# CVMI-Lab/DODA

Hardware: AMD Instinct MI355X
Metric: active-voxels/sec fwd+bwd SparseConv U-Net, ScanNet 2cm (higher is better)
Workload: dtype bf16; 1 GPU; cfgs/scannet SparseConv U-Net training step (voxel pooling + fwd + CE + bwd + SGD), 2 cm voxels, 4 scenes/GPU x ~150000 active voxels, random-init weights; global_batch=4, voxels_per_gpu=601279, points_per_gpu=781042, parallelism=dp1, n_classes=20, grad_sync=deferred multi-layer wgrad + bucketed all-reduce, collectives=none (single process), prefetch_gate=off, grad_exchange=no process group

## Files before the change

doda_amd/csrc/spconv_wdma.hip:

```cpp
#include "tilebook.hpp"
#include "spconv_common.hpp"
#include "wgrad_common.hpp"
#include <stdlib.h>
#include <type_traits>
#include <string.h>

namespace {

constexpr int WD_WAVES = 16;
constexpr int WD_ROWS_BYTES = (TB_UMAX + 1) * 32;
constexpr int WD_LIDX_BYTES = TB_LIDX_BYTES;
constexpr int WD_DY_BYTES = TB_T * 32;
constexpr int WD_UNITS_BYTES = 2 * TB_K * 256 * 4;
constexpr int WD_BUF_BYTES = (WD_ROWS_BYTES + WD_LIDX_BYTES + WD_DY_BYTES) > WD_UNITS_BYTES ? (WD_ROWS_BYTES + WD_LIDX_BYTES + WD_DY_BYTES)
                                                                                           : WD_UNITS_BYTES;
static_assert(WD_LIDX_BYTES % 1024 == 0, "whole DMA pieces");
constexpr int WD_UNITS = 2 * TB_K;
constexpr int WD_MAX_UNITS = (WD_UNITS + WD_WAVES - 1) / WD_WAVES;
constexpr int WD_MAX_JOBS = 16;
static_assert(WD_BUF_BYTES % 16 == 0 && 2 * WD_BUF_BYTES + 64 <= 160 * 1024, "two tile buffers per CU");
static_assert(WD_UNITS * 256 * 4 <= WD_BUF_BYTES, "the final exchange re-uses ONE tile buffer (the other may be a DMA target)");

struct WdJob { const void *x, *dy; float *part; unsigned x_stride, dy_stride; int first_rank, pad; };
struct WdJobs { int n; WdJob j[WD_MAX_JOBS]; };

__device__ __forceinline__ u32x4 wd_rsrc(const void *p, unsigned bytes) {
    const unsigned long long a = (unsigned long long)p;
    u32x4 r;
    r[0] = (unsigned)a;
    r[1] = (unsigned)(a >> 32) & 0xffffu;
    r[2] = bytes;
    r[3] = 0x00020000u;
    return r;
}
__device__ __forceinline__ void wd_dma16(unsigned lds_base, unsigned voff, const u32x4 &rs) {
    unsigned keep;
    asm volatile("s_mov_b32 %0, m0\n\t"
                 "s_mov_b32 m0, %1\n\t"
                 "s_nop 0\n\t"
                 "buffer_load_dwordx4 %2, %3, 0 offen lds\n\t"
                 "s_mov_b32 m0, %0"
                 : "=&s"(keep) : "s"(lds_base), "v"(voff), "s"(rs) : "memory");
}
__device__ __forceinline__ void wd_aload128(u32x4 &dst, unsigned voff, const u32x4 &rs) {
    asm volatile("buffer_load_dwordx4 %0, %1, %2, 0 offen" : "=v"(dst) : "v"(voff), "s"(rs) : "memory");
}
template <int TAG = 0>
__device__ __forceinline__ s16x4 wd_tr_b64(unsigned addr) {
    s16x4 v;
    asm volatile("ds_read_b64_tr_b16 %0, %1 ; %2" : "=v"(v) : "v"(addr), "n"(TAG) : "memory");
    return v;
}
__global__ __launch_bounds__(1024) void wgrad_dma16(const WdJobs jobs, const int32_t *__restrict__ tbl,
                                                    int ld, int n, const TileBookView tb) {
    __shared__ __attribute__((aligned(16))) unsigned char smem[2 * WD_BUF_BYTES];
    const int tid = threadIdx.x, wid = __builtin_amdgcn_readfirstlane(tid >> 6);
    const int lane = tid & 63, i = lane & 15, g = lane >> 4;
    const u32x4 rs_ul = wd_rsrc(tb.ulist, (unsigned)tb.nt * (unsigned)TB_UMAX * 4u);
    const u32x4 rs_li = wd_rsrc(tb.lidx, (unsigned)tb.nt * (unsigned)TB_LIDX_BYTES);

    const int G = gridDim.x, nt = tb.nt;
    const int rank = (int)(blockIdx.x & 7) * (G >> 3) + (int)(blockIdx.x >> 3);
    const long long N = (long long)jobs.n * nt;
    const int start = (int)((long long)rank * N / G), n_items = (int)((long long)(rank + 1) * N / G) - start;
    if (n_items == 0) return;

    if (tid < 4) reinterpret_cast<u32x4 *>(smem + (tid >> 1) * WD_BUF_BYTES)[tid & 1] = (u32x4){0u, 0u, 0u, 0u};

    const unsigned smem_base = (unsigned)(uintptr_t)smem;
    const unsigned src_half = (unsigned)(lane & 1) * 16u;
    const int w8 = wid & 7, kb = (wid >> 3) * 2;
    struct Where { int job; unsigned tile; bool ok; };
    auto where = [&](int item) {
        Where q;
        q.ok = item < n_items;
        const int gid = start + (q.ok ? item : 0);
        q.job = gid / nt;
        q.tile = (unsigned)(gid - q.job * nt);
        return q;
    };
    auto issue_list = [&](const Where &q, u32x2 &rid) {
        asm volatile("buffer_load_dwordx2 %0, %1, %2, 0 offen" : "=v"(rid)
                     : "v"(q.ok ? q.tile * (unsigned)(TB_UMAX * 4) + (unsigned)((w8 * 32 + (lane >> 1)) * 4 + kb) * 4u : OOB), "s"(rs_ul)
                     : "memory");
    };
    auto issue_rows = [&](const Where &q, int item, int k, const u32x2 &rid) {
        const unsigned buf = smem_base + (unsigned)(item & 1) * (unsigned)WD_BUF_BYTES;
        const unsigned xs = jobs.j[q.job].x_stride;
        const u32x4 rs_x = wd_rsrc(jobs.j[q.job].x, (unsigned)n * xs - (xs - 32u));
        if (!q.ok || __builtin_amdgcn_readfirstlane((int)rid[k]) < 0) return;
        wd_dma16(buf + 32u + (unsigned)(((kb + k) * 8 + w8) * 1024), rid[k] * xs + src_half, rs_x);
    };
    auto issue_strip = [&](const Where &q, int item) {
        const unsigned buf = smem_base + (unsigned)(item & 1) * (unsigned)WD_BUF_BYTES;
        if (wid < WD_LIDX_BYTES / 1024)
            wd_dma16(buf + (unsigned)WD_ROWS_BYTES + (unsigned)(wid * 1024),
                     q.ok ? q.tile * (unsigned)TB_LIDX_BYTES + (unsigned)(wid * 64 + lane) * 16u : OOB, rs_li);
    };
    auto issue_dy = [&](const Where &q, int item) {
        if (wid < 8) {
            const unsigned buf = smem_base + (unsigned)(item & 1) * (unsigned)WD_BUF_BYTES;
            const unsigned ds = jobs.j[q.job].dy_stride;
            const u32x4 rs_dy = wd_rsrc(jobs.j[q.job].dy, (unsigned)n * ds - (ds - 32u));
            wd_dma16(buf + (unsigned)(WD_ROWS_BYTES + WD_LIDX_BYTES) + (unsigned)(wid * 1024),
                     q.ok ? (q.tile * (unsigned)TB_T + (unsigned)(wid * 32 + (lane >> 1))) * ds + (unsigned)(lane & 1) * 16u : OOB, rs_dy);
        }
    };

    f32x4 acc[WD_MAX_UNITS];
#pragma unroll
    for (int m = 0; m < WD_MAX_UNITS; ++m) acc[m] = (f32x4){0.f, 0.f, 0.f, 0.f};
    const f32x4 zero = {0.f, 0.f, 0.f, 0.f};

    u32x2 la, lb;
    {
        const Where q0 = where(0), q1 = where(1);
        issue_list(q0, la);
        issue_list(q1, lb);
        asm volatile("s_waitcnt vmcnt(0)" : "+v"(la), "+v"(lb) : : "memory");
        asm volatile("s_waitcnt lgkmcnt(0)\n\ts_barrier" ::: "memory");
        issue_rows(q0, 0, 0, la);
        issue_rows(q0, 0, 1, la);
        issue_strip(q0, 0);
        issue_dy(q0, 0);
    }

    auto body = [&](int item, bool no_list, const u32x2 &lnext, u32x2 &lnew) {
        const Where qc = where(item), q1 = where(item + 1), q2 = where(item + 2);
        const int t0 = (int)qc.tile * TB_T;
        const unsigned char *buf = smem + (item & 1) * WD_BUF_BYTES;
        const unsigned rows_base = smem_base + (unsigned)(item & 1) * (unsigned)WD_BUF_BYTES;
        const unsigned *lidx_s = reinterpret_cast<const unsigned *>(buf + WD_ROWS_BYTES);
        const unsigned dy_base = rows_base + (unsigned)(WD_ROWS_BYTES + WD_LIDX_BYTES);
        const unsigned short *xg = reinterpret_cast<const unsigned short *>(jobs.j[qc.job].x);
        issue_list(q2, lnew);
        const int q4 = i >> 2, c4 = i & 3, hw = wid & 1;
        bf16x8 bt[4];
#pragma unroll
        for (int kk = 0; kk < 4; ++kk) {
            const unsigned a = dy_base + (unsigned)((32 * (4 * hw + kk) + 8 * g + q4) * 32 + c4 * 8);
            const s16x4 lo4 = wd_tr_b64(a), hi4 = wd_tr_b64(a + 4u * 32u);
            bt[kk] = __builtin_bit_cast(bf16x8, __builtin_shufflevector(lo4, hi4, 0, 1, 2, 3, 4, 5, 6, 7));
        }
        asm volatile("s_waitcnt lgkmcnt(0)" : "+v"(bt[0]), "+v"(bt[1]), "+v"(bt[2]), "+v"(bt[3]) : : "memory");
        const int rl = 8 * (i >> 2) + 4 * (g >> 1) + (i & 3);
        const unsigned hsel = (unsigned)(g & 1);
        if (!no_list) {
            const unsigned lane_off = rows_base + (unsigned)c4 * 8u;
            const bool tail_unit = wid + WD_WAVES * (WD_MAX_UNITS - 1) < WD_UNITS;
#pragma unroll
            for (int mp = 0; mp < WD_MAX_UNITS / 2; ++mp) {
                unsigned ra[8], rb[8];
#pragma unroll
                for (int mm = 0; mm < 2; ++mm) {
                    const int unit = wid + WD_WAVES * (2 * mp + mm);
                    const int o = unit < WD_UNITS ? unit >> 1 : 0;
#pragma unroll
                    for (int kp = 0; kp < 2; ++kp) {
                        const unsigned *sp = lidx_s + tb_lplane(o) * TB_T + tb_lpos((2 * hw + kp) * 64 + 8 * g + q4);
                        const unsigned shb = tb_lshift(o);
                        ra[mm * 4 + 2 * kp] = (__builtin_amdgcn_ubfe(sp[0], shb, 10u) << 5) + lane_off;
                        ra[mm * 4 + 2 * kp + 1] = (__builtin_amdgcn_ubfe(sp[2], shb, 10u) << 5) + lane_off;
                        rb[mm * 4 + 2 * kp] = (__builtin_amdgcn_ubfe(sp[32], shb, 10u) << 5) + lane_off;
                        rb[mm * 4 + 2 * kp + 1] = (__builtin_amdgcn_ubfe(sp[34], shb, 10u) << 5) + lane_off;
                    }
                }
                __builtin_amdgcn_sched_barrier(0);
                auto run_pair = [&](auto tagc) {
                    constexpr int TAG = decltype(tagc)::value;
                    constexpr int last = TAG == 1 ? 4 : 8;
                    s16x4 xl[3], xh[3];
                    xl[0] = wd_tr_b64<TAG>(ra[0]); xh[0] = wd_tr_b64<TAG>(rb[0]);
                    xl[1] = wd_tr_b64<TAG>(ra[1]); xh[1] = wd_tr_b64<TAG>(rb[1]);
#pragma unroll
                    for (int st = 0; st < last; ++st) {
                        const int gs = mp * 8 + st, m = gs >> 2, kk = gs & 3;
                        if (gs == (wid & 1)) issue_rows(q1, item + 1, 0, lnext);
                        if (gs == 2 + (wid & 1)) issue_rows(q1, item + 1, 1, lnext);
                        if (gs == 4 + (wid & 1)) issue_strip(q1, item + 1);
                        if (gs == 6 + (wid & 1)) issue_dy(q1, item + 1);
                        if (st + 2 < last) { xl[(st + 2) % 3] = wd_tr_b64<TAG>(ra[st + 2]); xh[(st + 2) % 3] = wd_tr_b64<TAG>(rb[st + 2]); }
                        const int newer = st + 2 < last ? 4 : 2 * (last - 1 - st);
                        if (newer == 4) asm volatile("s_waitcnt lgkmcnt(4)" : "+v"(xl[st % 3]), "+v"(xh[st % 3]) : : "memory");
                        else if (newer == 2) asm volatile("s_waitcnt lgkmcnt(2)" : "+v"(xl[st % 3]), "+v"(xh[st % 3]) : : "memory");
                        else asm volatile("s_waitcnt lgkmcnt(0)" : "+v"(xl[st % 3]), "+v"(xh[st % 3]) : : "memory");
                        const bf16x8 a = __builtin_bit_cast(bf16x8, __builtin_shufflevector(xl[st % 3], xh[st % 3], 0, 1, 2, 3, 4, 5, 6, 7));
                        acc[m] = __builtin_amdgcn_mfma_f32_16x16x32_bf16(a, bt[kk], acc[m], 0, 0, 0);
                        __builtin_amdgcn_sched_barrier(0);
                    }
                };
                if (mp < WD_MAX_UNITS / 2 - 1 || tail_unit) run_pair(std::integral_constant<int, 0>{});
                else run_pair(std::integral_constant<int, 1>{});
            }
        } else {
            issue_rows(q1, item + 1, 0, lnext);
            issue_rows(q1, item + 1, 1, lnext);
            issue_strip(q1, item + 1);
            issue_dy(q1, item + 1);
            bf16x8 P[2];
#pragma unroll
            for (int G = 0; G < 2; ++G) {
                u32x4 v = {0u, 0u, 0u, 0u};
                const bool mine = (g >> 1) == G && (i >> 3) == (g & 1);
                const int q = i & 7;
#pragma unroll
                for (int w = 0; w < 4; ++w) v[w] = (mine && (q >> 1) == w) ? ((q & 1) ? 0x3F800000u : 0x00003F80u) : 0u;
                P[G] = __builtin_bit_cast(bf16x8, v);
            }
#pragma unroll 1
            for (int m = 0; m < WD_MAX_UNITS; ++m) {
                const int unit = wid + WD_WAVES * m;
                if (unit >= WD_UNITS) break;
                const int o = unit >> 1;
                f32x4 part = {0.f, 0.f, 0.f, 0.f};
                int gi[4];
#pragma unroll
                for (int kk = 0; kk < 4; ++kk) {
                    const int r = 32 * (4 * hw + kk) + rl;
                    gi[kk] = t0 + r < n ? tbl[(size_t)o * ld + (size_t)(t0 + r)] : -1;
                }
                u32x4 v[4];
#pragma unroll
                for (int kk = 0; kk < 4; ++kk) {
                    v[kk] = (u32x4){0u, 0u, 0u, 0u};
                    if (gi[kk] >= 0) v[kk] = *reinterpret_cast<const u32x4 *>(xg + (size_t)gi[kk] * (jobs.j[qc.job].x_stride >> 1) + hsel * 8);
                }
#pragma unroll
                for (int kk = 0; kk < 4; ++kk) {
                    const bf16x8 a = __builtin_bit_cast(bf16x8, v[kk]);
                    const f32x4 e0 = __builtin_amdgcn_mfma_f32_16x16x32_bf16(a, P[0], zero, 0, 0, 0);
                    const f32x4 e1 = __builtin_amdgcn_mfma_f32_16x16x32_bf16(a, P[1], zero, 0, 0, 0);
                    part = __builtin_amdgcn_mfma_f32_16x16x32_bf16(pack_hi16(e0, e1), bt[kk], part, 0, 0, 0);
                }
#pragma unroll
                for (int mm = 0; mm < WD_MAX_UNITS; ++mm)
                    if (mm == m) acc[mm] += part;
            }
        }
    };

    auto flush = [&](int job, int bufsel, int last_gid) {
        asm volatile("s_waitcnt lgkmcnt(0)\n\ts_barrier" ::: "memory");
        float *ex = reinterpret_cast<float *>(smem + bufsel * WD_BUF_BYTES);
#pragma unroll
        for (int m = 0; m < WD_MAX_UNITS; ++m) {
            const int unit = wid + WD_WAVES * m;
            if (unit < WD_UNITS) {
#pragma unroll
                for (int r = 0; r < 4; ++r) ex[unit * 256 + (4 * g + r) * 16 + i] = acc[m][r];
            }
            acc[m] = (f32x4){0.f, 0.f, 0.f, 0.f};
        }
        asm volatile("s_waitcnt lgkmcnt(0)\n\ts_barrier" ::: "memory");
        const int pslot = N >= G ? rank - jobs.j[job].first_rank : last_gid - job * nt;
        float *dst = jobs.j[job].part + (size_t)pslot * (TB_K * 256);
        for (int e = tid; e < TB_K * 256; e += 1024) {
            const int o = e >> 8, c = e & 255;
            dst[e] = ex[(2 * o) * 256 + c] + ex[(2 * o + 1) * 256 + c];
        }
        asm volatile("s_waitcnt lgkmcnt(0)\n\ts_barrier" ::: "memory");
        if (tid < 2) reinterpret_cast<u32x4 *>(smem + bufsel * WD_BUF_BYTES)[tid] = (u32x4){0u, 0u, 0u, 0u};
        asm volatile("s_waitcnt lgkmcnt(0)\n\ts_barrier" ::: "memory");
    };

    bool nl_cur = __builtin_amdgcn_readfirstlane((int)la[0]) == -2;
    for (int item = 0; item < n_items; item += 2) {
        asm volatile("s_waitcnt vmcnt(0)" : "+v"(lb) : : "memory");
        asm volatile("s_waitcnt lgkmcnt(0)\n\ts_barrier" ::: "memory");
        {
            const bool nl_next = __builtin_amdgcn_readfirstlane((int)lb[0]) == -2;
            body(item, nl_cur, lb, la);
            nl_cur = nl_next;
        }
        if (item + 1 == n_items || (start + item + 1) % nt == 0) flush((start + item) / nt, item & 1, start + item);
        if (item + 1 >= n_items) break;
        asm volatile("s_waitcnt vmcnt(0)" : "+v"(la) : : "memory");
        asm volatile("s_waitcnt lgkmcnt(0)\n\ts_barrier" ::: "memory");
        {
            const bool nl_next = __builtin_amdgcn_readfirstlane((int)la[0]) == -2;
            body(item + 1, nl_cur, la, lb);
            nl_cur = nl_next;
        }
        if (item + 2 == n_items || (start + item + 2) % nt == 0) flush((start + item + 1) / nt, (item + 1) & 1, start + item + 1);
    }
    asm volatile("s_waitcnt vmcnt(0)" ::: "memory");
}

struct WdRJob { const float *part; float *dw; int accumulate, ldo, ldc, n_part; };
struct WdRJobs { WdRJob j[WD_MAX_JOBS]; };

__global__ __launch_bounds__(512) void wgrad_dma_reduce(const WdRJobs jobs) {
    __shared__ float red[16][32];
    const WdRJob d = jobs.j[blockIdx.y];
    const int n_part = d.n_part;
    const int jx = threadIdx.x & 31, p = threadIdx.x >> 5;
    const int e = blockIdx.x * 32 + jx;
    float a[8];
#pragma unroll
    for (int q = 0; q < 8; ++q) a[q] = 0.f;
    int b = p;
    for (; b + 7 * 16 < n_part; b += 8 * 16) {
#pragma unroll
        for (int q = 0; q < 8; ++q) a[q] += d.part[(size_t)(b + q * 16) * (TB_K * 256) + e];
    }
    for (int q = 0; b < n_part; b += 16, ++q) a[q & 7] += d.part[(size_t)b * (TB_K * 256) + e];
    red[p][jx] = ((a[0] + a[1]) + (a[2] + a[3])) + ((a[4] + a[5]) + (a[6] + a[7]));
    doda_sync();
    if (p == 0) {
        float v = 0.f;
#pragma unroll
        for (int q = 0; q < 16; ++q) v += red[q][jx];
        float *dst = d.dw + (size_t)(e >> 8) * d.ldo + (size_t)((e >> 4) & 15) * d.ldc + (e & 15);
        *dst = d.accumulate ? *dst + v : v;
    }
}

static_assert(WP_TILE_ROWS == TB_T && WP_TILE_K == TB_K, "wgrad_plan.hpp restates these constants");

struct Block { const void *x, *dy; float *dw; int x_stride, dy_stride, ldo, ldc, accumulate; };
struct WdArgs { WdJobs jobs; WdRJobs red; };

}

namespace doda_wdma {

Plan plan(const doda_wgrad_job *jobs, const std::vector<int> &idx) {
    Plan p;
    std::vector<char> done(idx.size(), 0);
    for (size_t q = 0; q < idx.size(); ++q) {
        if (done[q]) continue;
        const doda_wgrad_job &j0 = jobs[idx[q]];
        Plan::Launch l{(int)p.order.size(), 0, 0, p.partial_bytes};
        for (size_t r = q; r < idx.size(); ++r) {
            const doda_wgrad_job &j = jobs[idx[r]];
            if (done[r] || j.tilebook != j0.tilebook || j.tbl != j0.tbl || j.n_rows != j0.n_rows || j.ld != j0.ld) continue;
            done[r] = 1;
            p.order.push_back(idx[r]);
            ++l.n_jobs;
            l.n_blocks += wdma_blocks(j);
        }
        p.partial_bytes += (size_t)l.n_blocks * wdma_block_partial_bytes(j0.n_rows);
        p.launches.push_back(l);
    }
    return p;
}

void write_desc(Plan &p, const doda_wgrad_job *jobs, char *part) {
    p.args.clear();
    for (const Plan::Launch &l : p.launches) {
        const doda_wgrad_job &j0 = jobs[p.order[l.first_job]];
        std::vector<Block> blocks;
        for (int r = 0; r < l.n_jobs; ++r) {
            const doda_wgrad_job &j = jobs[p.order[l.first_job + r]];
            const int es = 2;
            for (int ci = 0; ci < j.ca; ci += 16)
                for (int co = 0; co < j.cb; co += 16)
                    blocks.push_back(Block{(const char *)j.a + ci * es, (const char *)j.b + co * es, j.dw + (size_t)ci * j.cb + co,
                                           j.ca * es, j.cb * es, j.ca * j.cb, j.cb, (j.flags & DODA_WGRAD_ACCUMULATE) ? 1 : 0});
        }
        const int groups = wdma_groups(j0.n_rows), nt = (j0.n_rows + TB_T - 1) / TB_T;
        size_t used = l.part_off;
        for (int first = 0; first < l.n_blocks; first += WD_MAX_JOBS) {
            const int nj = l.n_blocks - first < WD_MAX_JOBS ? l.n_blocks - first : WD_MAX_JOBS;
            WdArgs a;
            ::memset(&a, 0, sizeof(a));
            a.jobs.n = nj;
            int first_rank[WD_MAX_JOBS], count[WD_MAX_JOBS];
            for (int k = 0; k < nj; ++k) { first_rank[k] = -1; count[k] = 0; }
            const long long N = (long long)nj * nt;
            if (N >= groups) {
                for (int r = 0; r < groups; ++r) {
                    const long long st = (long long)r * N / groups, en = (long long)(r + 1) * N / groups;
                    for (long long b = st / nt; b <= (en - 1) / nt; ++b) {
                        if (first_rank[b] < 0) first_rank[b] = r;
                        ++count[b];
                    }
                }
            } else {
                for (int k = 0; k < nj; ++k) { first_rank[k] = 0; count[k] = nt; }
            }
            for (int k = 0; k < nj; ++k) {
                const Block &b = blocks[first + k];
                float *pp = (float *)(part + used);
                used += (size_t)count[k] * TB_K * 256 * sizeof(float);
                a.jobs.j[k] = WdJob{b.x, b.dy, pp, (unsigned)b.x_stride, (unsigned)b.dy_stride, first_rank[k], 0};
                a.red.j[k] = WdRJob{pp, b.dw, b.accumulate, b.ldo, b.ldc, count[k]};
            }
            const unsigned char *bytes = (const unsigned char *)&a;
            p.args.insert(p.args.end(), bytes, bytes + sizeof(a));
        }
    }
}

int launch(const Plan &p, const doda_wgrad_job *jobs, hipStream_t s) {
    const WdArgs *a = (const WdArgs *)p.args.data();
    for (const Plan::Launch &l : p.launches) {
        const doda_wgrad_job &j0 = jobs[p.order[l.first_job]];
        const TileBookView tb = tilebook_view(const_cast<void *>(j0.tilebook), j0.n_rows);
        for (int first = 0; first < l.n_blocks; first += WD_MAX_JOBS, ++a) {
            doda_wgrad::trace("wgrad_dma16", wdma_groups(j0.n_rows), 1024, a->jobs.n);
            hipLaunchKernelGGL(wgrad_dma16, dim3(wdma_groups(j0.n_rows)), dim3(1024), 0, s, a->jobs, j0.tbl, j0.ld, j0.n_rows, tb);
            doda_wgrad::trace("wgrad_dma_reduce", TB_K * 256 / 32 * a->jobs.n, 512, a->jobs.n);
            hipLaunchKernelGGL(wgrad_dma_reduce, dim3(TB_K * 256 / 32, a->jobs.n), dim3(512), 0, s, a->red);
        }
    }
    return doda_check_launch();
}

}
```

doda_amd/csrc/wgrad_backends.hpp:

```cpp
#pragma once
#include "common.hpp"
#include "wgrad_plan.hpp"
#include <vector>

namespace doda_wgrad {
WgradSwitches &switches();
inline void trace(const char *name, unsigned grid, unsigned block, int jobs) {
    if (switches().trace) fprintf(stderr, "wgrad route=%s grid=%u block=%u jobs=%d\n", name, grid, block, jobs);
}
struct RJob {
    const float4 *partial;
    float4 *dw;
    long long n_quad;
    int R, blk_end, accumulate, pad;
};
__host__ __device__ inline int reduce_lanes(int R) {
    int rl = 1;
    while (rl < 16 && rl < R) rl *= 2;
    return rl;
}
inline int reduce_blocks(long long n_quad, int R) { return div_up(n_quad, 256 / reduce_lanes(R)); }
inline void push_reduce(std::vector<RJob> &list, int *blocks, const void *partial, const doda_wgrad_job &j, int R) {
    RJob d;
    d.partial = (const float4 *)partial;
    d.dw = (float4 *)j.dw;
    d.n_quad = (long long)j.K * j.ca * j.cb / 4;
    d.R = R;
    d.accumulate = (j.flags & DODA_WGRAD_ACCUMULATE) ? 1 : 0;
    d.pad = 0;
    d.blk_end = *blocks += reduce_blocks(d.n_quad, R);
    list.push_back(d);
}
}

namespace doda_pairs {
struct Plan {
    std::vector<int> idx;
    std::vector<size_t> part_off;
    struct Group { int ta, tb, first, count, blocks; };
    std::vector<Group> groups;
    std::vector<int> order, blk_end;
    size_t partial_bytes = 0, desc_bytes = 0;
    int n_reduce = 0;
};
Plan plan(const doda_wgrad_job *jobs, const std::vector<int> &idx);
void write_desc(const Plan &p, const doda_wgrad_job *jobs, char *part, void *desc, std::vector<doda_wgrad::RJob> &reduce,
                int *reduce_blocks);
int launch(const Plan &p, const void *desc_dev, hipStream_t s);
size_t desc_bytes_per_job();
}

namespace doda_wdma {
inline bool enabled() { return doda_wgrad::switches().wdma; }
inline void set_enabled(bool on) { doda_wgrad::switches().wdma = on; }
struct Plan {
    struct Launch { int first_job, n_jobs, n_blocks; size_t part_off; };
    std::vector<Launch> launches;
    std::vector<int> order;
    std::vector<unsigned char> args;
    size_t partial_bytes = 0;
};
Plan plan(const doda_wgrad_job *jobs, const std::vector<int> &idx);
void write_desc(Plan &p, const doda_wgrad_job *jobs, char *part);
int launch(const Plan &p, const doda_wgrad_job *jobs, hipStream_t s);
}

namespace doda_wwide {
struct Plan {
    std::vector<unsigned char> desc;
    int n = 0, wgs = 0, red_blocks = 0;
    size_t partial_bytes = 0, desc_bytes = 0;
};
Plan plan(const doda_wgrad_job *jobs, const std::vector<int> &idx);
void write_desc(const Plan &p, char *part, void *desc);
int launch(const Plan &p, const void *desc_dev, hipStream_t s);
size_t desc_bytes_per_job();
}
```

doda_amd/csrc/wgrad_plan.hpp:

```cpp
#pragma once
#include <stddef.h>
#include <stdint.h>
#include <stdio.h>
#include <stdlib.h>
#include "../../include/doda_hip.h"

constexpr int WP_RT = 64;
constexpr int WP_MAX_OGW = 7;
constexpr int WP_TILE_ROWS = 256;
constexpr int WP_TILE_K = 27;
constexpr int WP_PAIRS_MAX_K = 28;
constexpr int WP_SEG_TILE = 256;
constexpr int WP_RANGE_TILES = 8;
constexpr int WP_RANGE_ROWS = WP_SEG_TILE * WP_RANGE_TILES;
#define WW_SHAPES(X) X(3, 3) X(2, 4) X(2, 3) X(1, 5) X(1, 6) X(1, 7) X(1, 4) X(1, 3)
constexpr int WW_MAX_BLOCKS = 9, WW_MAX_TA = 3, WW_MAX_TB = 7;

struct WgradSwitches {
    int min_rows = 512;
    bool no33 = false;
    int t33 = 128;
    long long f32_split_rows = -1;
    int wdma_min_rows = 32768;
    bool no_pairs = false;
    bool wdma = true;
    bool trace = false;
};
inline WgradSwitches wgrad_switches_from_env() {
    const auto num = [](const char *e, long long dflt) { return e && *e ? atoll(e) : dflt; };
    const auto on = [](const char *e) { return e && e[0] == '1'; };
    const WgradSwitches d;
    return {(int)num(getenv("DODA_WGRAD_MIN_ROWS"), d.min_rows), on(getenv("DODA_WGRAD_NO33")), (int)num(getenv("DODA_WGRAD_T33"), d.t33),
            num(getenv("DODA_F32_WGRAD_SPLIT_ROWS"), d.f32_split_rows), (int)num(getenv("DODA_WDMA_MIN_ROWS"), d.wdma_min_rows),
            on(getenv("DODA_WGRAD_NO_PAIRS")), !on(getenv("DODA_NO_WDMA")), on(getenv("DODA_TRACE_WGRAD"))};
}

#define WP_PAIR_SHAPES(X) X(1, 1) X(2, 1) X(1, 2) X(2, 2)

constexpr size_t wp_align256(size_t x) { return (x + 255) / 256 * 256; }
constexpr int wp_div_up(long long a, long long b) { return (int)((a + b - 1) / b); }
inline bool wp_al16(const void *p) { return ((uintptr_t)p & 15) == 0; }
inline bool wp_accumulate(const doda_wgrad_job &j) { return (j.flags & DODA_WGRAD_ACCUMULATE) != 0; }

struct PairsGeo {
    int ta, tb, n_tag, n_tbg, n_og, n_range;
    bool direct;
    long long blocks;
    size_t partial_bytes;
};
inline PairsGeo pairs_geo(const doda_wgrad_job &j) {
    PairsGeo g;
    const int na = j.ca / 16, nb = j.cb / 16;
    g.ta = na >= 2 ? 2 : 1;
    g.tb = nb >= 2 ? 2 : 1;
    g.n_tag = wp_div_up(na, g.ta);
    g.n_tbg = wp_div_up(nb, g.tb);
    g.n_og = wp_div_up(j.K, 4);
    const long long rows = j.pair_seg ? (long long)j.pair_seg_nt * WP_SEG_TILE : (long long)j.pair_ld;
    g.n_range = wp_div_up(rows > 0 ? rows : 1, WP_RANGE_ROWS);
    g.direct = g.n_range == 1 && !wp_accumulate(j);
    g.blocks = (long long)g.n_range * g.n_og * g.n_tag * g.n_tbg;
    g.partial_bytes = g.direct ? 0 : wp_align256((size_t)g.n_range * j.K * j.ca * j.cb * 4);
    return g;
}
inline bool pairs_eligible(const doda_wgrad_job &j) {
    if (j.elem_bytes != 2 || j.ca <= 0 || j.cb <= 0 || (j.ca % 16) || (j.cb % 16) || j.K <= 0 || j.n_rows <= 0) return false;
    if (!j.a || !j.b || !j.dw || j.K > WP_PAIRS_MAX_K) return false;
    if (!j.pair_in || !j.pair_out || j.pair_ld <= 0 || j.n_a <= 0) return false;
    if (j.pair_num ? (!j.pair_seg || j.pair_seg_nt <= 0) : (j.pair_seg != nullptr || j.K != 1)) return false;
    if ((unsigned long long)j.n_a * j.ca * 2ull >= 0x3fffffffull) return false;
    if ((unsigned long long)j.n_rows * j.cb * 2ull >= 0x3fffffffull) return false;
    if (!wp_al16(j.a) || !wp_al16(j.b) || !wp_al16(j.dw)) return false;
    return pairs_geo(j).blocks <= 0x3fffffff;
}

inline int wdma_groups(int n_rows) {
    const int groups = (wp_div_up(n_rows, WP_TILE_ROWS) + 7) / 8 * 8;
    return groups > 256 ? 256 : groups;
}
inline int wdma_blocks(const doda_wgrad_job &j) { return (j.ca / 16) * (j.cb / 16); }
inline size_t wdma_block_partial_bytes(int n_rows) { return wp_align256((size_t)wdma_groups(n_rows) * WP_TILE_K * 256 * sizeof(float)); }
inline bool wdma_eligible(const doda_wgrad_job &j, const WgradSwitches &sw) {
    return j.tilebook && j.tbl && j.elem_bytes == 2 && j.ca % 16 == 0 && j.ca <= 64 && j.cb % 16 == 0 && j.cb <= 64 &&
           j.K == WP_TILE_K && j.n_rows > 0 && j.a && j.b && j.dw && j.n_a == j.n_rows && j.ld >= j.n_rows &&
           (size_t)j.n_rows * 128 < 0x7ffffff0ull && (size_t)j.K * j.ld * 4 < 0xffffffffull &&
           !(((uintptr_t)j.a | (uintptr_t)j.b | (uintptr_t)j.tilebook) & 15) && sw.wdma;
}

inline bool ww_shape(int ca, int cb, int *ta, int *tb) {
    const int A = ca / 16, B = cb / 16;
    int b = B;
    while (b > WW_MAX_TB || B % b) --b;
    int a = WW_MAX_TA;
    while (a > 1 && (A % a || a * b > WW_MAX_BLOCKS)) --a;
    bool known = false;
#define WW_KNOWN(X, Y) known |= (a == X && b == Y);
    WW_SHAPES(WW_KNOWN)
#undef WW_KNOWN
    *ta = a; *tb = b;
    return known;
}
inline bool wwide_eligible(const doda_wgrad_job &j) {
    int ta, tb;
    return j.tilebook && j.tbl && j.elem_bytes == 2 && j.K == WP_TILE_K && j.n_rows > 0 && j.a && j.b && j.dw &&
           j.ca % 16 == 0 && j.cb % 16 == 0 && j.ca >= 48 && j.cb >= 48 && j.ca <= 224 && j.cb <= 224 &&
           j.n_a == j.n_rows && j.ld >= j.n_rows && !(((uintptr_t)j.a | (uintptr_t)j.b | (uintptr_t)j.tilebook | (uintptr_t)j.dw) & 15) &&
           ww_shape(j.ca, j.cb, &ta, &tb);
}

enum WgradClass { J_SKIP = 0, J_ZERO = 1, J_DENSE = 2, J_PAIRS = 3, J_TILE = 4, J_WIDE = 5 };
inline int classify(const doda_wgrad_job &j, const WgradSwitches &sw) {
    if (j.n_rows == 0 && j.dw && j.K > 0 && j.ca > 0 && j.cb > 0) return wp_accumulate(j) ? J_SKIP : J_ZERO;
    if (wwide_eligible(j) && !pairs_eligible(j)) return J_WIDE;
    if (wdma_eligible(j, sw) && (j.n_rows >= sw.wdma_min_rows || !pairs_eligible(j))) return J_TILE;
    if (pairs_eligible(j) && (!sw.no_pairs || !j.tbl)) return J_PAIRS;
    return J_DENSE;
}

enum WgradPolicy : uint8_t { WP_BF16, WP_F32, WP_F32S };
struct DensePlan {
    int TA, TB, OGW, n_og, n_tag, n_tbg, R, rows_per_chunk, blocks;
    WgradPolicy policy;
    bool vok;
    int key;
};
inline bool dense_valid(const doda_wgrad_job &j) {
    return j.ca > 0 && j.cb > 0 && j.K > 0 && j.K <= 4 * WP_MAX_OGW && j.n_rows > 0 && j.ld >= j.n_rows && j.a && j.b && j.tbl && j.dw &&
           (j.elem_bytes == 2 || j.elem_bytes == 4);
}
inline bool dense_vok(const doda_wgrad_job &j) {
    return (size_t)j.ca * j.elem_bytes % 16 == 0 && (size_t)j.cb * j.elem_bytes % 16 == 0 && wp_al16(j.a) && wp_al16(j.b);
}
inline DensePlan plan_dense(int K, int ca, int cb, int n_rows, int esz, bool vok, const WgradSwitches &sw) {
    DensePlan p;
    const int ta = (ca + 15) / 16, tb = (cb + 15) / 16;
    p.TA = (ta % 2 == 0) ? 2 : 1;
    p.TB = (tb % 2 == 0) ? 2 : 1;
    if (ta == 3 && tb == 3 && esz == 2 && K > 8 && !sw.no33) { p.TA = 3; p.TB = 3; }
    p.n_tag = ta / p.TA;
    p.n_tbg = tb / p.TB;
    p.OGW = (p.TA * p.TB == 4 || esz == 2) ? 4 : WP_MAX_OGW;
    if (p.TA * p.TB == 9 || K <= 8) p.OGW = 2;
    p.n_og = wp_div_up(K, 4 * p.OGW);
    const int gy = p.n_tag * p.n_tbg * p.n_og;
    const int rows = n_rows > 0 ? n_rows : 1;
    int R = wp_div_up(p.TA * p.TB == 9 ? sw.t33 : 512, gy);
    const int max_r = rows / sw.min_rows > 1 ? rows / sw.min_rows : 1;
    if (R > max_r) R = max_r;
    if (R < 1) R = 1;
    p.rows_per_chunk = wp_div_up(wp_div_up(rows, R), WP_RT) * WP_RT;
    p.R = wp_div_up(rows, p.rows_per_chunk);
    p.blocks = p.R * gy;
    const bool split = esz == 4 && sw.f32_split_rows >= 0 && (long long)n_rows >= sw.f32_split_rows;
    p.policy = esz == 2 ? WP_BF16 : split ? WP_F32S : WP_F32;
    p.vok = vok;
    p.key = ((((esz * 4 + p.TA) * 4 + p.TB) * 8 + p.OGW) * 2 + (vok ? 1 : 0)) * 2 + (split ? 1 : 0);
    return p;
}
inline DensePlan plan_dense(const doda_wgrad_job &j, const WgradSwitches &sw) {
    return plan_dense(j.K, j.ca, j.cb, j.n_rows, j.elem_bytes, dense_vok(j), sw);
}
inline bool dense_needs_partial(const DensePlan &p, const doda_wgrad_job &j) { return p.R > 1 || wp_accumulate(j); }
inline size_t dense_partial_bytes(const DensePlan &p, const doda_wgrad_job &j) {
    return dense_needs_partial(p, j) ? wp_align256((size_t)p.R * j.K * j.ca * j.cb * 4) : 0;
}

struct WideGeo { int ta, tb, P, rpc, blocks; size_t partial_bytes; };
inline WideGeo wwide_geo(const doda_wgrad_job &j, const WgradSwitches &sw) {
    WideGeo g;
    const DensePlan p = plan_dense(j, sw);
    ww_shape(j.ca, j.cb, &g.ta, &g.tb);
    g.P = p.R; g.rpc = p.rows_per_chunk;
    g.blocks = (j.ca / (16 * g.ta)) * (j.cb / (16 * g.tb)) * g.P;
    g.partial_bytes = wp_align256((size_t)g.blocks * WP_TILE_K * 256 * g.ta * g.tb * 4);
    return g;
}

template <int TA_, int TB_, int OGW_> struct WgradTile { static constexpr int TA = TA_, TB = TB_, OGW = OGW_; };
template <class... T> struct WgradTiles {};
typedef WgradTiles<WgradTile<3, 3, 2>, WgradTile<1, 1, 2>, WgradTile<2, 1, 2>, WgradTile<1, 2, 2>, WgradTile<2, 2, 2>, WgradTile<1, 1, 4>,
                   WgradTile<2, 1, 4>, WgradTile<1, 2, 4>, WgradTile<1, 1, 7>, WgradTile<2, 1, 7>, WgradTile<1, 2, 7>, WgradTile<2, 2, 4>> DenseTiles;
template <class... T>
constexpr bool wgrad_listed(WgradTiles<T...>, int ta, int tb, int ogw) { return ((T::TA == ta && T::TB == tb && T::OGW == ogw) || ...); }
constexpr bool dense_compiled(WgradPolicy p, int ta, int tb, int ogw) {
    return wgrad_listed(DenseTiles{}, ta, tb, ogw) && (p == WP_BF16 ? ogw != WP_MAX_OGW : ta * tb != 9 && (ogw == 2 || (ogw == 4) == (ta * tb == 4)));
}

inline int dense_name(const DensePlan &p, char *buf, size_t n) {
    static const char *const pol[3] = {"BF16", "F32", "F32S"};
    return snprintf(buf, n, "wgrad_multi_kernel<%s, %d, %d, %d, %s>", pol[p.policy], p.TA, p.TB, p.OGW, p.vok ? "true" : "false");
}
```

Measured before the change: 138.7 million voxels/s.

## Pair adjacent output-channel blocks in DMA wgrad kernel to reuse gathered input rows

Moves the wgrad DMA kernel into a header template with a PAIR mode. In that mode one workgroup computes two adjacent 16-wide output-channel blocks of the same layer and input, so each gathered x tile loaded into LDS feeds two MFMA accumulators instead of one. The aim is to halve the x gather and LDS transpose-read traffic per output block. The cost is more accumulator registers and a second exchange in the flush, which may lower occupancy. It is on by default and can be turned off with DODA_WDMA_PAIR.

Result: no change. 140.0 million voxels/s, median of 6 (+1.0%).

```diff
diff --git a/doda_amd/csrc/spconv_wdma.hip b/doda_amd/csrc/spconv_wdma.hip
--- a/doda_amd/csrc/spconv_wdma.hip
+++ b/doda_amd/csrc/spconv_wdma.hip
@@ -1,290 +1,6 @@
-#include "tilebook.hpp"
-#include "spconv_common.hpp"
-#include "wgrad_common.hpp"
-#include <stdlib.h>
-#include <type_traits>
-#include <string.h>
+#include "wdma_kernel.hpp"
 
 namespace {
-
-constexpr int WD_WAVES = 16;
-constexpr int WD_ROWS_BYTES = (TB_UMAX + 1) * 32;
-constexpr int WD_LIDX_BYTES = TB_LIDX_BYTES;
-constexpr int WD_DY_BYTES = TB_T * 32;
-constexpr int WD_UNITS_BYTES = 2 * TB_K * 256 * 4;
-constexpr int WD_BUF_BYTES = (WD_ROWS_BYTES + WD_LIDX_BYTES + WD_DY_BYTES) > WD_UNITS_BYTES ? (WD_ROWS_BYTES + WD_LIDX_BYTES + WD_DY_BYTES)
-                                                                                           : WD_UNITS_BYTES;
-static_assert(WD_LIDX_BYTES % 1024 == 0, "whole DMA pieces");
-constexpr int WD_UNITS = 2 * TB_K;
-constexpr int WD_MAX_UNITS = (WD_UNITS + WD_WAVES - 1) / WD_WAVES;
-constexpr int WD_MAX_JOBS = 16;
-static_assert(WD_BUF_BYTES % 16 == 0 && 2 * WD_BUF_BYTES + 64 <= 160 * 1024, "two tile buffers per CU");
-static_assert(WD_UNITS * 256 * 4 <= WD_BUF_BYTES, "the final exchange re-uses ONE tile buffer (the other may be a DMA target)");
-
-struct WdJob { const void *x, *dy; float *part; unsigned x_stride, dy_stride; int first_rank, pad; };
-struct WdJobs { int n; WdJob j[WD_MAX_JOBS]; };
-
-__device__ __forceinline__ u32x4 wd_rsrc(const void *p, unsigned bytes) {
-    const unsigned long long a = (unsigned long long)p;
-    u32x4 r;
-    r[0] = (unsigned)a;
-    r[1] = (unsigned)(a >> 32) & 0xffffu;
-    r[2] = bytes;
-    r[3] = 0x00020000u;
-    return r;
-}
-__device__ __forceinline__ void wd_dma16(unsigned lds_base, unsigned voff, const u32x4 &rs) {
-    unsigned keep;
-    asm volatile("s_mov_b32 %0, m0\n\t"
-                 "s_mov_b32 m0, %1\n\t"
-                 "s_nop 0\n\t"
-                 "buffer_load_dwordx4 %2, %3, 0 offen lds\n\t"
-                 "s_mov_b32 m0, %0"
-                 : "=&s"(keep) : "s"(lds_base), "v"(voff), "s"(rs) : "memory");
-}
-__device__ __forceinline__ void wd_aload128(u32x4 &dst, unsigned voff, const u32x4 &rs) {
-    asm volatile("buffer_load_dwordx4 %0, %1, %2, 0 offen" : "=v"(dst) : "v"(voff), "s"(rs) : "memory");
-}
-template <int TAG = 0>
-__device__ __forceinline__ s16x4 wd_tr_b64(unsigned addr) {
-    s16x4 v;
-    asm volatile("ds_read_b64_tr_b16 %0, %1 ; %2" : "=v"(v) : "v"(addr), "n"(TAG) : "memory");
-    return v;
-}
-__global__ __launch_bounds__(1024) void wgrad_dma16(const WdJobs jobs, const int32_t *__restrict__ tbl,
-                                                    int ld, int n, const TileBookView tb) {
-    __shared__ __attribute__((aligned(16))) unsigned char smem[2 * WD_BUF_BYTES];
-    const int tid = threadIdx.x, wid = __builtin_amdgcn_readfirstlane(tid >> 6);
-    const int lane = tid & 63, i = lane & 15, g = lane >> 4;
-    const u32x4 rs_ul = wd_rsrc(tb.ulist, (unsigned)tb.nt * (unsigned)TB_UMAX * 4u);
-    const u32x4 rs_li = wd_rsrc(tb.lidx, (unsigned)tb.nt * (unsigned)TB_LIDX_BYTES);
-
-    const int G = gridDim.x, nt = tb.nt;
-    const int rank = (int)(blockIdx.x & 7) * (G >> 3) + (int)(blockIdx.x >> 3);
-    const long long N = (long long)jobs.n * nt;
-    const int start = (int)((long long)rank * N / G), n_items = (int)((long long)(rank + 1) * N / G) - start;
-    if (n_items == 0) return;
-
-    if (tid < 4) reinterpret_cast<u32x4 *>(smem + (tid >> 1) * WD_BUF_BYTES)[tid & 1] = (u32x4){0u, 0u, 0u, 0u};
-
-    const unsigned smem_base = (unsigned)(uintptr_t)smem;
-    const unsigned src_half = (unsigned)(lane & 1) * 16u;
-    const int w8 = wid & 7, kb = (wid >> 3) * 2;
-    struct Where { int job; unsigned tile; bool ok; };
-    auto where = [&](int item) {
-        Where q;
-        q.ok = item < n_items;
-        const int gid = start + (q.ok ? item : 0);
-        q.job = gid / nt;
-        q.tile = (unsigned)(gid - q.job * nt);
-        return q;
-    };
-    auto issue_list = [&](const Where &q, u32x2 &rid) {
-        asm volatile("buffer_load_dwordx2 %0, %1, %2, 0 offen" : "=v"(rid)
-                     : "v"(q.ok ? q.tile * (unsigned)(TB_UMAX * 4) + (unsigned)((w8 * 32 + (lane >> 1)) * 4 + kb) * 4u : OOB), "s"(rs_ul)
-                     : "memory");
-    };
-    auto issue_rows = [&](const Where &q, int item, int k, const u32x2 &rid) {
-        const unsigned buf = smem_base + (unsigned)(item & 1) * (unsigned)WD_BUF_BYTES;
-        const unsigned xs = jobs.j[q.job].x_stride;
-        const u32x4 rs_x = wd_rsrc(jobs.j[q.job].x, (unsigned)n * xs - (xs - 32u));
-        if (!q.ok || __builtin_amdgcn_readfirstlane((int)rid[k]) < 0) return;
-        wd_dma16(buf + 32u + (unsigned)(((kb + k) * 8 + w8) * 1024), rid[k] * xs + src_half, rs_x);
-    };
-    auto issue_strip = [&](const Where &q, int item) {
-        const unsigned buf = smem_base + (unsigned)(item & 1) * (unsigned)WD_BUF_BYTES;
-        if (wid < WD_LIDX_BYTES / 1024)
-            wd_dma16(buf + (unsigned)WD_ROWS_BYTES + (unsigned)(wid * 1024),
-                     q.ok ? q.tile * (unsigned)TB_LIDX_BYTES + (unsigned)(wid * 64 + lane) * 16u : OOB, rs_li);
-    };
-    auto issue_dy = [&](const Where &q, int item) {
-        if (wid < 8) {
-            const unsigned buf = smem_base + (unsigned)(item & 1) * (unsigned)WD_BUF_BYTES;
-            const unsigned ds = jobs.j[q.job].dy_stride;
-            const u32x4 rs_dy = wd_rsrc(jobs.j[q.job].dy, (unsigned)n * ds - (ds - 32u));
-            wd_dma16(buf + (unsigned)(WD_ROWS_BYTES + WD_LIDX_BYTES) + (unsigned)(wid * 1024),
-                     q.ok ? (q.tile * (unsigned)TB_T + (unsigned)(wid * 32 + (lane >> 1))) * ds + (unsigned)(lane & 1) * 16u : OOB, rs_dy);
-        }
-    };
-
-    f32x4 acc[WD_MAX_UNITS];
-#pragma unroll
-    for (int m = 0; m < WD_MAX_UNITS; ++m) acc[m] = (f32x4){0.f, 0.f, 0.f, 0.f};
-    const f32x4 zero = {0.f, 0.f, 0.f, 0.f};
-
-    u32x2 la, lb;
-    {
-        const Where q0 = where(0), q1 = where(1);
-        issue_list(q0, la);
-        issue_list(q1, lb);
-        asm volatile("s_waitcnt vmcnt(0)" : "+v"(la), "+v"(lb) : : "memory");
-        asm volatile("s_waitcnt lgkmcnt(0)\n\ts_barrier" ::: "memory");
-        issue_rows(q0, 0, 0, la);
-        issue_rows(q0, 0, 1, la);
-        issue_strip(q0, 0);
-        issue_dy(q0, 0);
-    }
-
-    auto body = [&](int item, bool no_list, const u32x2 &lnext, u32x2 &lnew) {
-        const Where qc = where(item), q1 = where(item + 1), q2 = where(item + 2);
-        const int t0 = (int)qc.tile * TB_T;
-        const unsigned char *buf = smem + (item & 1) * WD_BUF_BYTES;
-        const unsigned rows_base = smem_base + (unsigned)(item & 1) * (unsigned)WD_BUF_BYTES;
-        const unsigned *lidx_s = reinterpret_cast<const unsigned *>(buf + WD_ROWS_BYTES);
-        const unsigned dy_base = rows_base + (unsigned)(WD_ROWS_BYTES + WD_LIDX_BYTES);
-        const unsigned short *xg = reinterpret_cast<const unsigned short *>(jobs.j[qc.job].x);
-        issue_list(q2, lnew);
-        const int q4 = i >> 2, c4 = i & 3, hw = wid & 1;
-        bf16x8 bt[4];
-#pragma unroll
-        for (int kk = 0; kk < 4; ++kk) {
-            const unsigned a = dy_base + (unsigned)((32 * (4 * hw + kk) + 8 * g + q4) * 32 + c4 * 8);
-            const s16x4 lo4 = wd_tr_b64(a), hi4 = wd_tr_b64(a + 4u * 32u);
-            bt[kk] = __builtin_bit_cast(bf16x8, __builtin_shufflevector(lo4, hi4, 0, 1, 2, 3, 4, 5, 6, 7));
-        }
-        asm volatile("s_waitcnt lgkmcnt(0)" : "+v"(bt[0]), "+v"(bt[1]), "+v"(bt[2]), "+v"(bt[3]) : : "memory");
-        const int rl = 8 * (i >> 2) + 4 * (g >> 1) + (i & 3);
-        const unsigned hsel = (unsigned)(g & 1);
-        if (!no_list) {
-            const unsigned lane_off = rows_base + (unsigned)c4 * 8u;
-            const bool tail_unit = wid + WD_WAVES * (WD_MAX_UNITS - 1) < WD_UNITS;
-#pragma unroll
-            for (int mp = 0; mp < WD_MAX_UNITS / 2; ++mp) {
-                unsigned ra[8], rb[8];
-#pragma unroll
-                for (int mm = 0; mm < 2; ++mm) {
-                    const int unit = wid + WD_WAVES * (2 * mp + mm);
-                    const int o = unit < WD_UNITS ? unit >> 1 : 0;
-#pragma unroll
-                    for (int kp = 0; kp < 2; ++kp) {
-                        const unsigned *sp = lidx_s + tb_lplane(o) * TB_T + tb_lpos((2 * hw + kp) * 64 + 8 * g + q4);
-                        const unsigned shb = tb_lshift(o);
-                        ra[mm * 4 + 2 * kp] = (__builtin_amdgcn_ubfe(sp[0], shb, 10u) << 5) + lane_off;
-                        ra[mm * 4 + 2 * kp + 1] = (__builtin_amdgcn_ubfe(sp[2], shb, 10u) << 5) + lane_off;
-                        rb[mm * 4 + 2 * kp] = (__builtin_amdgcn_ubfe(sp[32], shb, 10u) << 5) + lane_off;
-                        rb[mm * 4 + 2 * kp + 1] = (__builtin_amdgcn_ubfe(sp[34], shb, 10u) << 5) + lane_off;
-                    }
-                }
-                __builtin_amdgcn_sched_barrier(0);
-                auto run_pair = [&](auto tagc) {
-                    constexpr int TAG = decltype(tagc)::value;
-                    constexpr int last = TAG == 1 ? 4 : 8;
-                    s16x4 xl[3], xh[3];
-                    xl[0] = wd_tr_b64<TAG>(ra[0]); xh[0] = wd_tr_b64<TAG>(rb[0]);
-                    xl[1] = wd_tr_b64<TAG>(ra[1]); xh[1] = wd_tr_b64<TAG>(rb[1]);
-#pragma unroll
-                    for (int st = 0; st < last; ++st) {
-                        const int gs = mp * 8 + st, m = gs >> 2, kk = gs & 3;
-                        if (gs == (wid & 1)) issue_rows(q1, item + 1, 0, lnext);
-                        if (gs == 2 + (wid & 1)) issue_rows(q1, item + 1, 1, lnext);
-                        if (gs == 4 + (wid & 1)) issue_strip(q1, item + 1);
-                        if (gs == 6 + (wid & 1)) issue_dy(q1, item + 1);
-                        if (st + 2 < last) { xl[(st + 2) % 3] = wd_tr_b64<TAG>(ra[st + 2]); xh[(st + 2) % 3] = wd_tr_b64<TAG>(rb[st + 2]); }
-                        const int newer = st + 2 < last ? 4 : 2 * (last - 1 - st);
-                        if (newer == 4) asm volatile("s_waitcnt lgkmcnt(4)" : "+v"(xl[st % 3]), "+v"(xh[st % 3]) : : "memory");
-                        else if (newer == 2) asm volatile("s_waitcnt lgkmcnt(2)" : "+v"(xl[st % 3]), "+v"(xh[st % 3]) : : "memory");
-                        else asm volatile("s_waitcnt lgkmcnt(0)" : "+v"(xl[st % 3]), "+v"(xh[st % 3]) : : "memory");
-                        const bf16x8 a = __builtin_bit_cast(bf16x8, __builtin_shufflevector(xl[st % 3], xh[st % 3], 0, 1, 2, 3, 4, 5, 6, 7));
-                        acc[m] = __builtin_amdgcn_mfma_f32_16x16x32_bf16(a, bt[kk], acc[m], 0, 0, 0);
-                        __builtin_amdgcn_sched_barrier(0);
-                    }
-                };
-                if (mp < WD_MAX_UNITS / 2 - 1 || tail_unit) run_pair(std::integral_constant<int, 0>{});
-                else run_pair(std::integral_constant<int, 1>{});
-            }
-        } else {
-            issue_rows(q1, item + 1, 0, lnext);
-            issue_rows(q1, item + 1, 1, lnext);
-            issue_strip(q1, item + 1);
-            issue_dy(q1, item + 1);
-            bf16x8 P[2];
-#pragma unroll
-            for (int G = 0; G < 2; ++G) {
-                u32x4 v = {0u, 0u, 0u, 0u};
-                const bool mine = (g >> 1) == G && (i >> 3) == (g & 1);
-                const int q = i & 7;
-#pragma unroll
-                for (int w = 0; w < 4; ++w) v[w] = (mine && (q >> 1) == w) ? ((q & 1) ? 0x3F800000u : 0x00003F80u) : 0u;
-                P[G] = __builtin_bit_cast(bf16x8, v);
-            }
-#pragma unroll 1
-            for (int m = 0; m < WD_MAX_UNITS; ++m) {
-                const int unit = wid + WD_WAVES * m;
-                if (unit >= WD_UNITS) break;
-                const int o = unit >> 1;
-                f32x4 part = {0.f, 0.f, 0.f, 0.f};
-                int gi[4];
-#pragma unroll
-                for (int kk = 0; kk < 4; ++kk) {
-                    const int r = 32 * (4 * hw + kk) + rl;
-                    gi[kk] = t0 + r < n ? tbl[(size_t)o * ld + (size_t)(t0 + r)] : -1;
-                }
-                u32x4 v[4];
-#pragma unroll
-                for (int kk = 0; kk < 4; ++kk) {
-                    v[kk] = (u32x4){0u, 0u, 0u, 0u};
-                    if (gi[kk] >= 0) v[kk] = *reinterpret_cast<const u32x4 *>(xg + (size_t)gi[kk] * (jobs.j[qc.job].x_stride >> 1) + hsel * 8);
-                }
-#pragma unroll
-                for (int kk = 0; kk < 4; ++kk) {
-                    const bf16x8 a = __builtin_bit_cast(bf16x8, v[kk]);
-                    const f32x4 e0 = __builtin_amdgcn_mfma_f32_16x16x32_bf16(a, P[0], zero, 0, 0, 0);
-                    const f32x4 e1 = __builtin_amdgcn_mfma_f32_16x16x32_bf16(a, P[1], zero, 0, 0, 0);
-                    part = __builtin_amdgcn_mfma_f32_16x16x32_bf16(pack_hi16(e0, e1), bt[kk], part, 0, 0, 0);
-                }
-#pragma unroll
-                for (int mm = 0; mm < WD_MAX_UNITS; ++mm)
-                    if (mm == m) acc[mm] += part;
-            }
-        }
-    };
-
-    auto flush = [&](int job, int bufsel, int last_gid) {
-        asm volatile("s_waitcnt lgkmcnt(0)\n\ts_barrier" ::: "memory");
-        float *ex = reinterpret_cast<float *>(smem + bufsel * WD_BUF_BYTES);
-#pragma unroll
-        for (int m = 0; m < WD_MAX_UNITS; ++m) {
-            const int unit = wid + WD_WAVES * m;
-            if (unit < WD_UNITS) {
-#pragma unroll
-                for (int r = 0; r < 4; ++r) ex[unit * 256 + (4 * g + r) * 16 + i] = acc[m][r];
-            }
-            acc[m] = (f32x4){0.f, 0.f, 0.f, 0.f};
-        }
-        asm volatile("s_waitcnt lgkmcnt(0)\n\ts_barrier" ::: "memory");
-        const int pslot = N >= G ? rank - jobs.j[job].first_rank : last_gid - job * nt;
-        float *dst = jobs.j[job].part + (size_t)pslot * (TB_K * 256);
-        for (int e = tid; e < TB_K * 256; e += 1024) {
-            const int o = e >> 8, c = e & 255;
-            dst[e] = ex[(2 * o) * 256 + c] + ex[(2 * o + 1) * 256 + c];
-        }
-        asm volatile("s_waitcnt lgkmcnt(0)\n\ts_barrier" ::: "memory");
-        if (tid < 2) reinterpret_cast<u32x4 *>(smem + bufsel * WD_BUF_BYTES)[tid] = (u32x4){0u, 0u, 0u, 0u};
-        asm volatile("s_waitcnt lgkmcnt(0)\n\ts_barrier" ::: "memory");
-    };
-
-    bool nl_cur = __builtin_amdgcn_readfirstlane((int)la[0]) == -2;
-    for (int item = 0; item < n_items; item += 2) {
-        asm volatile("s_waitcnt vmcnt(0)" : "+v"(lb) : : "memory");
-        asm volatile("s_waitcnt lgkmcnt(0)\n\ts_barrier" ::: "memory");
-        {
-            const bool nl_next = __builtin_amdgcn_readfirstlane((int)lb[0]) == -2;
-            body(item, nl_cur, lb, la);
-            nl_cur = nl_next;
-        }
-        if (item + 1 == n_items || (start + item + 1) % nt == 0) flush((start + item) / nt, item & 1, start + item);
-        if (item + 1 >= n_items) break;
-        asm volatile("s_waitcnt vmcnt(0)" : "+v"(la) : : "memory");
-        asm volatile("s_waitcnt lgkmcnt(0)\n\ts_barrier" ::: "memory");
-        {
-            const bool nl_next = __builtin_amdgcn_readfirstlane((int)la[0]) == -2;
-            body(item + 1, nl_cur, la, lb);
-            nl_cur = nl_next;
-        }
-        if (item + 2 == n_items || (start + item + 2) % nt == 0) flush((start + item + 1) / nt, (item + 1) & 1, start + item + 1);
-    }
-    asm volatile("s_waitcnt vmcnt(0)" ::: "memory");
-}
 
 struct WdRJob { const float *part; float *dw; int accumulate, ldo, ldc, n_part; };
 struct WdRJobs { WdRJob j[WD_MAX_JOBS]; };
@@ -317,8 +33,13 @@
 
 static_assert(WP_TILE_ROWS == TB_T && WP_TILE_K == TB_K, "wgrad_plan.hpp restates these constants");
 
-struct Block { const void *x, *dy; float *dw; int x_stride, dy_stride, ldo, ldc, accumulate; };
-struct WdArgs { WdJobs jobs; WdRJobs red; };
+struct Block { const void *x, *dy; float *dw; int x_stride, dy_stride, ldo, ldc, accumulate, layer; };
+struct WdArgs { WdJobs jobs; WdRJobs red; int n_blocks, any_pair; };
+
+bool wd_pairable(const Block &a, const Block &b) {
+    return a.layer == b.layer && a.x == b.x && a.x_stride == b.x_stride && (const char *)b.dy == (const char *)a.dy + 32 &&
+           a.dy_stride == b.dy_stride;
+}
 
 }
 
@@ -356,7 +77,7 @@
             for (int ci = 0; ci < j.ca; ci += 16)
                 for (int co = 0; co < j.cb; co += 16)
                     blocks.push_back(Block{(const char *)j.a + ci * es, (const char *)j.b + co * es, j.dw + (size_t)ci * j.cb + co,
-                                           j.ca * es, j.cb * es, j.ca * j.cb, j.cb, (j.flags & DODA_WGRAD_ACCUMULATE) ? 1 : 0});
+                                           j.ca * es, j.cb * es, j.ca * j.cb, j.cb, (j.flags & DODA_WGRAD_ACCUMULATE) ? 1 : 0, r});
         }
         const int groups = wdma_groups(j0.n_rows), nt = (j0.n_rows + TB_T - 1) / TB_T;
         size_t used = l.part_off;
@@ -364,10 +85,19 @@
             const int nj = l.n_blocks - first < WD_MAX_JOBS ? l.n_blocks - first : WD_MAX_JOBS;
             WdArgs a;
             ::memset(&a, 0, sizeof(a));
-            a.jobs.n = nj;
+            int head[WD_MAX_JOBS], ni = 0;
+            bool two[WD_MAX_JOBS];
+            for (int k = 0; k < nj; ++ni) {
+                head[ni] = k;
+                two[ni] = doda_wgrad::switches().wdma_pair && k + 1 < nj && wd_pairable(blocks[first + k], blocks[first + k + 1]);
+                a.any_pair |= two[ni] ? 1 : 0;
+                k += two[ni] ? 2 : 1;
+            }
+            a.n_blocks = nj;
+            a.jobs.n = ni;
             int first_rank[WD_MAX_JOBS], count[WD_MAX_JOBS];
-            for (int k = 0; k < nj; ++k) { first_rank[k] = -1; count[k] = 0; }
-            const long long N = (long long)nj * nt;
+            for (int k = 0; k < ni; ++k) { first_rank[k] = -1; count[k] = 0; }
+            const long long N = (long long)ni * nt;
             if (N >= groups) {
                 for (int r = 0; r < groups; ++r) {
                     const long long st = (long long)r * N / groups, en = (long long)(r + 1) * N / groups;
@@ -377,14 +107,18 @@
                     }
                 }
             } else {
-                for (int k = 0; k < nj; ++k) { first_rank[k] = 0; count[k] = nt; }
+                for (int k = 0; k < ni; ++k) { first_rank[k] = 0; count[k] = nt; }
             }
-            for (int k = 0; k < nj; ++k) {
-                const Block &b = blocks[first + k];
-                float *pp = (float *)(part + used);
-                used += (size_t)count[k] * TB_K * 256 * sizeof(float);
-                a.jobs.j[k] = WdJob{b.x, b.dy, pp, (unsigned)b.x_stride, (unsigned)b.dy_stride, first_rank[k], 0};
-                a.red.j[k] = WdRJob{pp, b.dw, b.accumulate, b.ldo, b.ldc, count[k]};
+            for (int k = 0; k < ni; ++k) {
+                float *pp[2] = {nullptr, nullptr};
+                for (int h = 0; h < (two[k] ? 2 : 1); ++h) {
+                    const Block &b = blocks[first + head[k] + h];
+                    pp[h] = (float *)(part + used);
+                    used += (size_t)count[k] * TB_K * 256 * sizeof(float);
+                    a.red.j[head[k] + h] = WdRJob{pp[h], b.dw, b.accumulate, b.ldo, b.ldc, count[k]};
+                }
+                const Block &b = blocks[first + head[k]];
+                a.jobs.j[k] = WdJob{b.x, b.dy, pp[0], pp[1], (unsigned)b.x_stride, (unsigned)b.dy_stride, first_rank[k], 0};
             }
             const unsigned char *bytes = (const unsigned char *)&a;
             p.args.insert(p.args.end(), bytes, bytes + sizeof(a));
@@ -398,10 +132,13 @@
         const doda_wgrad_job &j0 = jobs[p.order[l.first_job]];
         const TileBookView tb = tilebook_view(const_cast<void *>(j0.tilebook), j0.n_rows);
         for (int first = 0; first < l.n_blocks; first += WD_MAX_JOBS, ++a) {
-            doda_wgrad::trace("wgrad_dma16", wdma_groups(j0.n_rows), 1024, a->jobs.n);
-            hipLaunchKernelGGL(wgrad_dma16, dim3(wdma_groups(j0.n_rows)), dim3(1024), 0, s, a->jobs, j0.tbl, j0.ld, j0.n_rows, tb);
-            doda_wgrad::trace("wgrad_dma_reduce", TB_K * 256 / 32 * a->jobs.n, 512, a->jobs.n);
-            hipLaunchKernelGGL(wgrad_dma_reduce, dim3(TB_K * 256 / 32, a->jobs.n), dim3(512), 0, s, a->red);
+            doda_wgrad::trace("wgrad_dma16", wdma_groups(j0.n_rows), 1024, a->n_blocks);
+            if (a->any_pair)
+                launch_pair(wdma_groups(j0.n_rows), &a->jobs, j0.tbl, j0.ld, j0.n_rows, tb, s);
+            else
+                hipLaunchKernelGGL(wgrad_dma16<false>, dim3(wdma_groups(j0.n_rows)), dim3(1024), 0, s, a->jobs, j0.tbl, j0.ld, j0.n_rows, tb);
+            doda_wgrad::trace("wgrad_dma_reduce", TB_K * 256 / 32 * a->n_blocks, 512, a->n_blocks);
+            hipLaunchKernelGGL(wgrad_dma_reduce, dim3(TB_K * 256 / 32, a->n_blocks), dim3(512), 0, s, a->red);
         }
     }
     return doda_check_launch();
diff --git a/doda_amd/csrc/spconv_wdma_pair.hip b/doda_amd/csrc/spconv_wdma_pair.hip
--- /dev/null
+++ b/doda_amd/csrc/spconv_wdma_pair.hip
@@ -0,0 +1,9 @@
+#include "wdma_kernel.hpp"
+
+namespace doda_wdma {
+
+void launch_pair(int groups, const void *wd_jobs, const int32_t *tbl, int ld, int n_rows, const TileBookView &tb, hipStream_t s) {
+    hipLaunchKernelGGL(wgrad_dma16<true>, dim3(groups), dim3(1024), 0, s, *static_cast<const WdJobs *>(wd_jobs), tbl, ld, n_rows, tb);
+}
+
+}
diff --git a/doda_amd/csrc/wdma_kernel.hpp b/doda_amd/csrc/wdma_kernel.hpp
--- /dev/null
+++ b/doda_amd/csrc/wdma_kernel.hpp
@@ -0,0 +1,333 @@
+#pragma once
+#include "tilebook.hpp"
+#include "spconv_common.hpp"
+#include "wgrad_common.hpp"
+#include <stdlib.h>
+#include <type_traits>
+#include <string.h>
+
+namespace {
+
+constexpr int WD_WAVES = 16;
+constexpr int WD_ROWS_BYTES = (TB_UMAX + 1) * 32;
+constexpr int WD_LIDX_BYTES = TB_LIDX_BYTES;
+constexpr int WD_DY_BYTES = TB_T * 32;
+constexpr int WD_UNITS_BYTES = 2 * TB_K * 256 * 4;
+constexpr int wd_buf_bytes(bool pair) {
+    const int staged = WD_ROWS_BYTES + WD_LIDX_BYTES + (pair ? 2 : 1) * WD_DY_BYTES;
+    return staged > WD_UNITS_BYTES ? staged : WD_UNITS_BYTES;
+}
+static_assert(WD_LIDX_BYTES % 1024 == 0, "whole DMA pieces");
+constexpr int WD_UNITS = 2 * TB_K;
+constexpr int WD_MAX_UNITS = (WD_UNITS + WD_WAVES - 1) / WD_WAVES;
+constexpr int WD_MAX_JOBS = 16;
+static_assert(wd_buf_bytes(false) % 16 == 0 && wd_buf_bytes(true) % 16 == 0 && 2 * wd_buf_bytes(true) + 64 <= 160 * 1024, "two tile buffers per CU");
+static_assert(WD_UNITS * 256 * 4 <= wd_buf_bytes(false), "the final exchange re-uses ONE tile buffer (the other may be a DMA target)");
+
+struct WdJob { const void *x, *dy; float *part, *part2; unsigned x_stride, dy_stride; int first_rank, pad; };
+struct WdJobs { int n; WdJob j[WD_MAX_JOBS]; };
+
+__device__ __forceinline__ u32x4 wd_rsrc(const void *p, unsigned bytes) {
+    const unsigned long long a = (unsigned long long)p;
+    u32x4 r;
+    r[0] = (unsigned)a;
+    r[1] = (unsigned)(a >> 32) & 0xffffu;
+    r[2] = bytes;
+    r[3] = 0x00020000u;
+    return r;
+}
+__device__ __forceinline__ void wd_dma16(unsigned lds_base, unsigned voff, const u32x4 &rs) {
+    unsigned keep;
+    asm volatile("s_mov_b32 %0, m0\n\t"
+                 "s_mov_b32 m0, %1\n\t"
+                 "s_nop 0\n\t"
+                 "buffer_load_dwordx4 %2, %3, 0 offen lds\n\t"
+                 "s_mov_b32 m0, %0"
+                 : "=&s"(keep) : "s"(lds_base), "v"(voff), "s"(rs) : "memory");
+}
+__device__ __forceinline__ void wd_aload128(u32x4 &dst, unsigned voff, const u32x4 &rs) {
+    asm volatile("buffer_load_dwordx4 %0, %1, %2, 0 offen" : "=v"(dst) : "v"(voff), "s"(rs) : "memory");
+}
+template <int TAG = 0>
+__device__ __forceinline__ s16x4 wd_tr_b64(unsigned addr) {
+    s16x4 v;
+    asm volatile("ds_read_b64_tr_b16 %0, %1 ; %2" : "=v"(v) : "v"(addr), "n"(TAG) : "memory");
+    return v;
+}
+template <bool PAIR>
+__global__ __launch_bounds__(1024) void wgrad_dma16(const WdJobs jobs, const int32_t *__restrict__ tbl,
+                                                    int ld, int n, const TileBookView tb) {
+    constexpr int WD_BUF_BYTES = wd_buf_bytes(PAIR);
+    __shared__ __attribute__((aligned(16))) unsigned char smem[2 * WD_BUF_BYTES];
+    const int tid = threadIdx.x, wid = __builtin_amdgcn_readfirstlane(tid >> 6);
+    int lane = tid & 63;
+    const u32x4 rs_ul = wd_rsrc(tb.ulist, (unsigned)tb.nt * (unsigned)TB_UMAX * 4u);
+    const u32x4 rs_li = wd_rsrc(tb.lidx, (unsigned)tb.nt * (unsigned)TB_LIDX_BYTES);
+
+    const int G = gridDim.x, nt = tb.nt;
+    const int rank = (int)(blockIdx.x & 7) * (G >> 3) + (int)(blockIdx.x >> 3);
+    const long long N = (long long)jobs.n * nt;
+    const int start = (int)((long long)rank * N / G), n_items = (int)((long long)(rank + 1) * N / G) - start;
+    if (n_items == 0) return;
+
+    if (tid < 4) reinterpret_cast<u32x4 *>(smem + (tid >> 1) * WD_BUF_BYTES)[tid & 1] = (u32x4){0u, 0u, 0u, 0u};
+
+    const unsigned smem_base = (unsigned)(uintptr_t)smem;
+    const int w8 = wid & 7, kb = (wid >> 3) * 2;
+    struct Where { int job; unsigned tile; bool ok; };
+    auto where = [&](int item) {
+        Where q;
+        q.ok = item < n_items;
+        const int gid = start + (q.ok ? item : 0);
+        q.job = gid / nt;
+        q.tile = (unsigned)(gid - q.job * nt);
+        return q;
+    };
+    auto issue_list = [&](const Where &q, u32x2 &rid) {
+        asm volatile("buffer_load_dwordx2 %0, %1, %2, 0 offen" : "=v"(rid)
+                     : "v"(q.ok ? q.tile * (unsigned)(TB_UMAX * 4) + (unsigned)((w8 * 32 + (lane >> 1)) * 4 + kb) * 4u : OOB), "s"(rs_ul)
+                     : "memory");
+    };
+    auto issue_rows = [&](const Where &q, int item, int k, const u32x2 &rid) {
+        const unsigned buf = smem_base + (unsigned)(item & 1) * (unsigned)WD_BUF_BYTES;
+        const unsigned xs = jobs.j[q.job].x_stride;
+        const u32x4 rs_x = wd_rsrc(jobs.j[q.job].x, (unsigned)n * xs - (xs - 32u));
+        if (!q.ok || __builtin_amdgcn_readfirstlane((int)rid[k]) < 0) return;
+        wd_dma16(buf + 32u + (unsigned)(((kb + k) * 8 + w8) * 1024), rid[k] * xs + (unsigned)(lane & 1) * 16u, rs_x);
+    };
+    auto issue_strip = [&](const Where &q, int item) {
+        const unsigned buf = smem_base + (unsigned)(item & 1) * (unsigned)WD_BUF_BYTES;
+        if (wid < WD_LIDX_BYTES / 1024)
+            wd_dma16(buf + (unsigned)WD_ROWS_BYTES + (unsigned)(wid * 1024),
+                     q.ok ? q.tile * (unsigned)TB_LIDX_BYTES + (unsigned)(wid * 64 + lane) * 16u : OOB, rs_li);
+    };
+    auto issue_dy = [&](const Where &q, int item) {
+        const unsigned second = (unsigned)(wid >> 3);
+        if (!second || (PAIR && jobs.j[q.job].part2 != nullptr)) {
+            const unsigned buf = smem_base + (unsigned)(item & 1) * (unsigned)WD_BUF_BYTES;
+            const unsigned ds = jobs.j[q.job].dy_stride;
+            const u32x4 rs_dy = wd_rsrc((const char *)jobs.j[q.job].dy + second * 32u, (unsigned)n * ds - (ds - 32u));
+            wd_dma16(buf + (unsigned)(WD_ROWS_BYTES + WD_LIDX_BYTES) + second * (unsigned)WD_DY_BYTES + (unsigned)(w8 * 1024),
+                     q.ok ? (q.tile * (unsigned)TB_T + (unsigned)(w8 * 32 + (lane >> 1))) * ds + (unsigned)(lane & 1) * 16u : OOB, rs_dy);
+        }
+    };
+
+    constexpr int N2 = PAIR ? WD_MAX_UNITS : 1;
+    f32x4 acc[WD_MAX_UNITS], acc2[N2];
+#pragma unroll
+    for (int m = 0; m < WD_MAX_UNITS; ++m) acc[m] = (f32x4){0.f, 0.f, 0.f, 0.f};
+#pragma unroll
+    for (int m = 0; m < N2; ++m) acc2[m] = (f32x4){0.f, 0.f, 0.f, 0.f};
+
+    u32x2 la, lb;
+    {
+        const Where q0 = where(0), q1 = where(1);
+        issue_list(q0, la);
+        issue_list(q1, lb);
+        asm volatile("s_waitcnt vmcnt(0)" : "+v"(la), "+v"(lb) : : "memory");
+        asm volatile("s_waitcnt lgkmcnt(0)\n\ts_barrier" ::: "memory");
+        issue_rows(q0, 0, 0, la);
+        issue_rows(q0, 0, 1, la);
+        issue_strip(q0, 0);
+        issue_dy(q0, 0);
+    }
+
+    auto body = [&](int item, bool no_list, const u32x2 &lnext, u32x2 &lnew) {
+        const Where qc = where(item), q1 = where(item + 1), q2 = where(item + 2);
+        if constexpr (PAIR) asm volatile("" : "+v"(lane));
+        const int i = lane & 15, g = lane >> 4;
+        const unsigned char *buf = smem + (item & 1) * WD_BUF_BYTES;
+        const unsigned rows_base = smem_base + (unsigned)(item & 1) * (unsigned)WD_BUF_BYTES;
+        const unsigned *lidx_s = reinterpret_cast<const unsigned *>(buf + WD_ROWS_BYTES);
+        const unsigned dy_base = rows_base + (unsigned)(WD_ROWS_BYTES + WD_LIDX_BYTES);
+        const unsigned short *xg = reinterpret_cast<const unsigned short *>(jobs.j[qc.job].x);
+        issue_list(q2, lnew);
+        const int q4 = i >> 2, c4 = i & 3, hw = wid & 1;
+        bf16x8 bt[4], bt2[PAIR ? 4 : 1];
+#pragma unroll
+        for (int kk = 0; kk < 4; ++kk) {
+            const unsigned a = dy_base + (unsigned)((32 * (4 * hw + kk) + 8 * g + q4) * 32 + c4 * 8);
+            const s16x4 lo4 = wd_tr_b64(a), hi4 = wd_tr_b64(a + 4u * 32u);
+            bt[kk] = __builtin_bit_cast(bf16x8, __builtin_shufflevector(lo4, hi4, 0, 1, 2, 3, 4, 5, 6, 7));
+            if constexpr (PAIR) {
+                const s16x4 lo2 = wd_tr_b64(a + (unsigned)WD_DY_BYTES), hi2 = wd_tr_b64(a + (unsigned)WD_DY_BYTES + 4u * 32u);
+                bt2[kk] = __builtin_bit_cast(bf16x8, __builtin_shufflevector(lo2, hi2, 0, 1, 2, 3, 4, 5, 6, 7));
+            }
+        }
+        if constexpr (PAIR)
+            asm volatile("s_waitcnt lgkmcnt(0)" : "+v"(bt[0]), "+v"(bt[1]), "+v"(bt[2]), "+v"(bt[3]), "+v"(bt2[0]), "+v"(bt2[1]), "+v"(bt2[2]),
+                         "+v"(bt2[3]) : : "memory");
+        else
+            asm volatile("s_waitcnt lgkmcnt(0)" : "+v"(bt[0]), "+v"(bt[1]), "+v"(bt[2]), "+v"(bt[3]) : : "memory");
+        const int rl = 8 * (i >> 2) + 4 * (g >> 1) + (i & 3);
+        const unsigned hsel = (unsigned)(g & 1);
+        if (!no_list) {
+            constexpr int UPP = PAIR ? 1 : 2;
+            const unsigned lane_off = rows_base + (unsigned)c4 * 8u;
+            const bool tail_unit = wid + WD_WAVES * (WD_MAX_UNITS - 1) < WD_UNITS;
+#pragma unroll
+            for (int mp = 0; mp < WD_MAX_UNITS / UPP; ++mp) {
+                unsigned ra[4 * UPP], rb[4 * UPP];
+#pragma unroll
+                for (int mm = 0; mm < UPP; ++mm) {
+                    const int unit = wid + WD_WAVES * (UPP * mp + mm);
+                    const int o = unit < WD_UNITS ? unit >> 1 : 0;
+#pragma unroll
+                    for (int kp = 0; kp < 2; ++kp) {
+                        const unsigned *sp = lidx_s + tb_lplane(o) * TB_T + tb_lpos((2 * hw + kp) * 64 + 8 * g + q4);
+                        const unsigned shb = tb_lshift(o);
+                        ra[mm * 4 + 2 * kp] = (__builtin_amdgcn_ubfe(sp[0], shb, 10u) << 5) + lane_off;
+                        ra[mm * 4 + 2 * kp + 1] = (__builtin_amdgcn_ubfe(sp[2], shb, 10u) << 5) + lane_off;
+                        rb[mm * 4 + 2 * kp] = (__builtin_amdgcn_ubfe(sp[32], shb, 10u) << 5) + lane_off;
+                        rb[mm * 4 + 2 * kp + 1] = (__builtin_amdgcn_ubfe(sp[34], shb, 10u) << 5) + lane_off;
+                    }
+                }
+                __builtin_amdgcn_sched_barrier(0);
+                auto run_pair = [&](auto tagc) {
+                    constexpr int TAG = decltype(tagc)::value;
+                    constexpr int last = TAG == 1 ? 4 : 4 * UPP;
+                    s16x4 xl[3], xh[3];
+                    xl[0] = wd_tr_b64<TAG>(ra[0]); xh[0] = wd_tr_b64<TAG>(rb[0]);
+                    xl[1] = wd_tr_b64<TAG>(ra[1]); xh[1] = wd_tr_b64<TAG>(rb[1]);
+#pragma unroll
+                    for (int st = 0; st < last; ++st) {
+                        const int gs = mp * 4 * UPP + st, m = gs >> 2, kk = gs & 3;
+                        if (gs == (wid & 1)) issue_rows(q1, item + 1, 0, lnext);
+                        if (gs == 2 + (wid & 1)) issue_rows(q1, item + 1, 1, lnext);
+                        if (gs == 4 + (wid & 1)) issue_strip(q1, item + 1);
+                        if (gs == 6 + (wid & 1)) issue_dy(q1, item + 1);
+                        if (st + 2 < last) { xl[(st + 2) % 3] = wd_tr_b64<TAG>(ra[st + 2]); xh[(st + 2) % 3] = wd_tr_b64<TAG>(rb[st + 2]); }
+                        const int newer = st + 2 < last ? 4 : 2 * (last - 1 - st);
+                        if (newer == 4) asm volatile("s_waitcnt lgkmcnt(4)" : "+v"(xl[st % 3]), "+v"(xh[st % 3]) : : "memory");
+                        else if (newer == 2) asm volatile("s_waitcnt lgkmcnt(2)" : "+v"(xl[st % 3]), "+v"(xh[st % 3]) : : "memory");
+                        else asm volatile("s_waitcnt lgkmcnt(0)" : "+v"(xl[st % 3]), "+v"(xh[st % 3]) : : "memory");
+                        const bf16x8 a = __builtin_bit_cast(bf16x8, __builtin_shufflevector(xl[st % 3], xh[st % 3], 0, 1, 2, 3, 4, 5, 6, 7));
+                        acc[m] = __builtin_amdgcn_mfma_f32_16x16x32_bf16(a, bt[kk], acc[m], 0, 0, 0);
+                        if constexpr (PAIR) acc2[m] = __builtin_amdgcn_mfma_f32_16x16x32_bf16(a, bt2[kk], acc2[m], 0, 0, 0);
+                        __builtin_amdgcn_sched_barrier(0);
+                    }
+                };
+                if (mp < WD_MAX_UNITS / UPP - 1 || tail_unit) run_pair(std::integral_constant<int, 0>{});
+                else if constexpr (UPP == 2) run_pair(std::integral_constant<int, 1>{});
+            }
+        } else {
+            issue_rows(q1, item + 1, 0, lnext);
+            issue_rows(q1, item + 1, 1, lnext);
+            issue_strip(q1, item + 1);
+            issue_dy(q1, item + 1);
+            f32x4 zero = {0.f, 0.f, 0.f, 0.f};
+            if constexpr (PAIR) asm volatile("" : "+v"(zero));
+            const int t0 = PAIR ? __builtin_amdgcn_readfirstlane((int)qc.tile * TB_T) : (int)qc.tile * TB_T;
+            bf16x8 P[2];
+#pragma unroll
+            for (int G = 0; G < 2; ++G) {
+                u32x4 v = {0u, 0u, 0u, 0u};
+                const bool mine = (g >> 1) == G && (i >> 3) == (g & 1);
+                const int q = i & 7;
+#pragma unroll
+                for (int w = 0; w < 4; ++w) v[w] = (mine && (q >> 1) == w) ? ((q & 1) ? 0x3F800000u : 0x00003F80u) : 0u;
+                P[G] = __builtin_bit_cast(bf16x8, v);
+            }
+#pragma unroll 1
+            for (int m = 0; m < WD_MAX_UNITS; ++m) {
+                const int unit = wid + WD_WAVES * m;
+                if (unit >= WD_UNITS) break;
+                const int o = unit >> 1;
+                f32x4 part = {0.f, 0.f, 0.f, 0.f}, part2 = {0.f, 0.f, 0.f, 0.f};
+                constexpr int KB = PAIR ? 2 : 4;
+#pragma unroll
+                for (int k0 = 0; k0 < 4; k0 += KB) {
+                    int gi[KB];
+#pragma unroll
+                    for (int kk = 0; kk < KB; ++kk) {
+                        const int r = 32 * (4 * hw + k0 + kk) + rl;
+                        gi[kk] = t0 + r < n ? tbl[(size_t)o * ld + (size_t)(t0 + r)] : -1;
+                    }
+                    u32x4 v[KB];
+#pragma unroll
+                    for (int kk = 0; kk < KB; ++kk) {
+                        v[kk] = (u32x4){0u, 0u, 0u, 0u};
+                        if (gi[kk] >= 0) v[kk] = *reinterpret_cast<const u32x4 *>(xg + (size_t)gi[kk] * (jobs.j[qc.job].x_stride >> 1) + hsel * 8);
+                    }
+#pragma unroll
+                    for (int kk = 0; kk < KB; ++kk) {
+                        const bf16x8 a = __builtin_bit_cast(bf16x8, v[kk]);
+                        const f32x4 e0 = __builtin_amdgcn_mfma_f32_16x16x32_bf16(a, P[0], zero, 0, 0, 0);
+                        const f32x4 e1 = __builtin_amdgcn_mfma_f32_16x16x32_bf16(a, P[1], zero, 0, 0, 0);
+                        const auto at = pack_hi16(e0, e1);
+                        part = __builtin_amdgcn_mfma_f32_16x16x32_bf16(at, bt[k0 + kk], part, 0, 0, 0);
+                        if constexpr (PAIR) part2 = __builtin_amdgcn_mfma_f32_16x16x32_bf16(at, bt2[k0 + kk], part2, 0, 0, 0);
+                    }
+                }
+#pragma unroll
+                for (int mm = 0; mm < WD_MAX_UNITS; ++mm)
+                    if (mm == m) acc[mm] += part;
+                if constexpr (PAIR) {
+#pragma unroll
+                    for (int mm = 0; mm < WD_MAX_UNITS; ++mm)
+                        if (mm == m) acc2[mm] += part2;
+                }
+            }
+        }
+    };
+
+    auto flush = [&](int job, int bufsel, int last_gid) {
+        asm volatile("s_waitcnt lgkmcnt(0)\n\ts_barrier" ::: "memory");
+        float *ex = reinterpret_cast<float *>(smem + bufsel * WD_BUF_BYTES);
+        const int i = lane & 15, g = lane >> 4;
+        const int ftid = PAIR ? wid * 64 + lane : tid;
+        const int pslot = N >= G ? rank - jobs.j[job].first_rank : last_gid - job * nt;
+        auto exchange = [&](f32x4 *av, float *part) {
+#pragma unroll
+            for (int m = 0; m < WD_MAX_UNITS; ++m) {
+                const int unit = wid + WD_WAVES * m;
+                if (unit < WD_UNITS) {
+#pragma unroll
+                    for (int r = 0; r < 4; ++r) ex[unit * 256 + (4 * g + r) * 16 + i] = av[m][r];
+                }
+                av[m] = (f32x4){0.f, 0.f, 0.f, 0.f};
+            }
+            asm volatile("s_waitcnt lgkmcnt(0)\n\ts_barrier" ::: "memory");
+            float *dst = part + (size_t)pslot * (TB_K * 256);
+            for (int e = ftid; e < TB_K * 256; e += 1024) {
+                const int o = e >> 8, c = e & 255;
+                dst[e] = ex[(2 * o) * 256 + c] + ex[(2 * o + 1) * 256 + c];
+            }
+            asm volatile("s_waitcnt lgkmcnt(0)\n\ts_barrier" ::: "memory");
+        };
+        exchange(acc, jobs.j[job].part);
+        if constexpr (PAIR) {
+            if (jobs.j[job].part2 != nullptr) exchange(acc2, jobs.j[job].part2);
+            else {
+#pragma unroll
+                for (int m = 0; m < WD_MAX_UNITS; ++m) acc2[m] = (f32x4){0.f, 0.f, 0.f, 0.f};
+            }
+        }
+        if (ftid < 2) reinterpret_cast<u32x4 *>(smem + bufsel * WD_BUF_BYTES)[ftid] = (u32x4){0u, 0u, 0u, 0u};
+        asm volatile("s_waitcnt lgkmcnt(0)\n\ts_barrier" ::: "memory");
+    };
+
+    bool nl_cur = __builtin_amdgcn_readfirstlane((int)la[0]) == -2;
+    for (int item = 0; item < n_items; item += 2) {
+        asm volatile("s_waitcnt vmcnt(0)" : "+v"(lb) : : "memory");
+        asm volatile("s_waitcnt lgkmcnt(0)\n\ts_barrier" ::: "memory");
+        {
+            const bool nl_next = __builtin_amdgcn_readfirstlane((int)lb[0]) == -2;
+            body(item, nl_cur, lb, la);
+            nl_cur = nl_next;
+        }
+        if (item + 1 == n_items || (start + item + 1) % nt == 0) flush((start + item) / nt, item & 1, start + item);
+        if (item + 1 >= n_items) break;
+        asm volatile("s_waitcnt vmcnt(0)" : "+v"(la) : : "memory");
+        asm volatile("s_waitcnt lgkmcnt(0)\n\ts_barrier" ::: "memory");
+        {
+            const bool nl_next = __builtin_amdgcn_readfirstlane((int)la[0]) == -2;
+            body(item + 1, nl_cur, la, lb);
+            nl_cur = nl_next;
+        }
+        if (item + 2 == n_items || (start + item + 2) % nt == 0) flush((start + item + 1) / nt, (item + 1) & 1, start + item + 1);
+    }
+    asm volatile("s_waitcnt vmcnt(0)" ::: "memory");
+}
+
+}
diff --git a/doda_amd/csrc/wgrad_backends.hpp b/doda_amd/csrc/wgrad_backends.hpp
--- a/doda_amd/csrc/wgrad_backends.hpp
+++ b/doda_amd/csrc/wgrad_backends.hpp
@@ -2,6 +2,8 @@
 #include "common.hpp"
 #include "wgrad_plan.hpp"
 #include <vector>
+
+struct TileBookView;
 
 namespace doda_wgrad {
 WgradSwitches &switches();
@@ -63,6 +65,7 @@
 Plan plan(const doda_wgrad_job *jobs, const std::vector<int> &idx);
 void write_desc(Plan &p, const doda_wgrad_job *jobs, char *part);
 int launch(const Plan &p, const doda_wgrad_job *jobs, hipStream_t s);
+void launch_pair(int groups, const void *wd_jobs, const int32_t *tbl, int ld, int n_rows, const TileBookView &tb, hipStream_t s);
 }
 
 namespace doda_wwide {
diff --git a/doda_amd/csrc/wgrad_plan.hpp b/doda_amd/csrc/wgrad_plan.hpp
--- a/doda_amd/csrc/wgrad_plan.hpp
+++ b/doda_amd/csrc/wgrad_plan.hpp
@@ -24,6 +24,7 @@
     int wdma_min_rows = 32768;
     bool no_pairs = false;
     bool wdma = true;
+    bool wdma_pair = true;
     bool trace = false;
 };
 inline WgradSwitches wgrad_switches_from_env() {
@@ -32,7 +33,8 @@
     const WgradSwitches d;
     return {(int)num(getenv("DODA_WGRAD_MIN_ROWS"), d.min_rows), on(getenv("DODA_WGRAD_NO33")), (int)num(getenv("DODA_WGRAD_T33"), d.t33),
             num(getenv("DODA_F32_WGRAD_SPLIT_ROWS"), d.f32_split_rows), (int)num(getenv("DODA_WDMA_MIN_ROWS"), d.wdma_min_rows),
-            on(getenv("DODA_WGRAD_NO_PAIRS")), !on(getenv("DODA_NO_WDMA")), on(getenv("DODA_TRACE_WGRAD"))};
+            on(getenv("DODA_WGRAD_NO_PAIRS")), !on(getenv("DODA_NO_WDMA")), num(getenv("DODA_WDMA_PAIR"), d.wdma_pair) != 0,
+            on(getenv("DODA_TRACE_WGRAD"))};
 }
 
 #define WP_PAIR_SHAPES(X) X(1, 1) X(2, 1) X(1, 2) X(2, 2)
```
